# Oneflow-Inc/libai

Hardware: AMD Instinct MI355X
Metric: tokens/sec (whole node), GPT-2 345M 3D-parallel at 1/2/4/8 MI355X (higher is better)
Workload: dtype bf16; 1 GPU; model=gpt2-345m (nl24 h1024 nah16 seq1024), global_batch=48, seq_len=1024, parallelism=dp1

## Files before the change

### libai_amd/csrc/bindings.cpp

```cpp
#include <algorithm>
#include <torch/extension.h>
#include <c10/hip/HIPStream.h>
#include <hip/hip_runtime_api.h>

#include <tuple>
#include <vector>

namespace {

hipStream_t cur_stream() { return c10::hip::getCurrentHIPStream().stream(); }

void check_launch(const char* name) {
  hipError_t err = hipGetLastError();
  TORCH_CHECK(err == hipSuccess, name, " launch failed: ", hipGetErrorString(err));
}

bool is_bf16(const torch::Tensor& t) {
  TORCH_CHECK(t.scalar_type() == torch::kBFloat16 || t.scalar_type() == torch::kFloat32,
              "libai_amd kernels support bf16/f32, got ", t.scalar_type());
  return t.scalar_type() == torch::kBFloat16;
}

void check_bias_width(const char* op, int W, int V) {
  TORCH_CHECK(W % V == 0 && W >= V, op, ": width ", W,
// ... 70 lines not shown
                    int64_t,
                    int64_t, int64_t, int64_t, int64_t, int64_t, int64_t, int64_t,
                    int64_t, int64_t, int64_t, int64_t, int64_t, int64_t, int64_t,
                    int64_t, int64_t, int64_t, int64_t, int64_t, int64_t, int64_t,
                    int64_t, int, int, int, int, int, float, float, uint64_t, int,
                    int, const float*, int, const float*, float*, const int*,
                    const int*, hipStream_t);
void attn_dropout_apply_bf16(void*, int64_t, int64_t, int64_t, float, uint64_t,
                             hipStream_t);
void attn_dropout_apply_f32(void*, int64_t, int64_t, int64_t, float, uint64_t,
                            hipStream_t);
void embedding_fwd_bf16(const int64_t*, const void*, void*, int64_t, int64_t,
                        int64_t, int64_t, hipStream_t);
void embedding_fwd_f32(const int64_t*, const void*, void*, int64_t, int64_t,
                       int64_t, int64_t, hipStream_t);
void embedding_bwd_bf16(const int64_t*, const void*, float*, int64_t, int64_t,
                        int64_t, int64_t, int64_t, hipStream_t);
void embedding_bwd_f32(const int64_t*, const void*, float*, int64_t, int64_t,
                       int64_t, int64_t, int64_t, hipStream_t);
void gemm_dw_bf16(const void*, const void*, float*, void*, int, int64_t, int64_t,
                  int64_t, int64_t, hipStream_t);
void flash_decode_bf16(const void*, const void*, const void*, void*, const int*,
                       int64_t, int64_t, int64_t, int64_t, int64_t, int64_t,
                       int64_t, int64_t, int64_t, int64_t, int, int, int, int,
                       float, int, const float*, int, hipStream_t);
int flash_decode_num_splits(int, int, int);
void flash_decode_split_bf16(const void*, const void*, const void*, void*,
                             float*, float*, float*, const int*, int64_t,
                             int64_t, int64_t, int64_t, int64_t, int64_t,
                             int64_t, int64_t, int64_t, int64_t, int, int, int,
                             int, int, float, int, const float*, int,
                             hipStream_t);
void rope_fwd_bf16(const void*, void*, const float*, const float*, int64_t, int64_t,
                   int64_t, int64_t, int64_t, int64_t, int, int, int, int, int,
                   const int*, int, hipStream_t);
void rope_fwd_f32(const void*, void*, const float*, const float*, int64_t, int64_t,
                  int64_t, int64_t, int64_t, int64_t, int, int, int, int, int,
                  const int*, int, hipStream_t);
void rope_bwd_bf16(const void*, void*, const float*, const float*, int64_t, int64_t,
                   int64_t, int64_t, int64_t, int64_t, int, int, int, int, int,
                   const int*, int, hipStream_t);
void rope_bwd_f32(const void*, void*, const float*, const float*, int64_t, int64_t,
                  int64_t, int64_t, int64_t, int64_t, int, int, int, int, int,
                  const int*, int, hipStream_t);
void rope_kv_insert_bf16(const void*, const void*, const void*, void*, void*,
                         void*, const float*, const float*, const long long*,
                         int, int, int, int, int64_t, int64_t, int64_t, int64_t,
                         int64_t, int64_t, int64_t, int, int, hipStream_t);
void quant_fp8_bf16(const void*, void*, const float*, float*, int64_t,
                    hipStream_t);
void res_ln_fwd_bf16(const void*, const void*, const void*, const void*,
                     const void*, void*, void*, int64_t, int, float, bool,
                     hipStream_t);
void swiglu_fwd_bf16(const void*, void*, int64_t, int, hipStream_t);
void swiglu_fwd_f32(const void*, void*, int64_t, int, hipStream_t);
void swiglu_bwd_bf16(const void*, const void*, void*, int64_t, int, hipStream_t);
void swiglu_bwd_f32(const void*, const void*, void*, int64_t, int, hipStream_t);
int adamw_chunk_elems();
void adamw_step_bf16(const void*, int, float, float, float, float, float, float, float,
                     float, hipStream_t);
void adamw_step_f32(const void*, int, float, float, float, float, float, float, float,
                    float, hipStream_t);
void l2norm_sq_bf16(const void*, int, float*, hipStream_t);
void l2norm_sq_f32(const void*, int, float*, hipStream_t);
}

std::tuple<torch::Tensor, torch::Tensor, torch::Tensor> ln_fwd(
    torch::Tensor x, torch::Tensor gamma, c10::optional<torch::Tensor> beta, bool rms,
    double eps) {
  CHECK_IN(x);
  CHECK_IN(gamma);
  const int H = (int)gamma.numel();
  const int64_t R = x.numel() / H;
  auto y = torch::empty_like(x);
  auto opts = x.options().dtype(torch::kFloat32);
  auto mean = rms ? torch::empty({0}, opts) : torch::empty({R}, opts);
  auto rstd = torch::empty({R}, opts);
  const void* bptr = nullptr;
  if (beta.has_value()) {
    CHECK_IN(beta.value());
    bptr = beta->data_ptr();
  }
  auto fn = is_bf16(x) ? ln_fwd_bf16 : ln_fwd_f32;
  fn(x.data_ptr(), gamma.data_ptr(), bptr, y.data_ptr(),
     rms ? nullptr : mean.data_ptr<float>(), rstd.data_ptr<float>(), R, H, (float)eps,
     rms, cur_stream());
  check_launch("ln_fwd");
  return {y, mean, rstd};
}

std::tuple<torch::Tensor, torch::Tensor, torch::Tensor> ln_bwd(
    torch::Tensor dy, torch::Tensor x, torch::Tensor gamma, torch::Tensor mean,
    torch::Tensor rstd, bool rms, bool need_dbeta) {
  CHECK_IN(dy);
  CHECK_IN(x);
  const int H = (int)gamma.numel();
  const int64_t R = x.numel() / H;
  auto dx = torch::empty_like(x);
  auto dgamma = torch::empty_like(gamma);
  auto dbeta = need_dbeta ? torch::empty_like(gamma) : torch::Tensor();
  const int64_t gxw = std::max<int64_t>(1, (H / 8 + 255) / 256);
  const int P = (int)std::min<int64_t>(std::max<int64_t>(1, 1024 / gxw),
                                       std::max<int64_t>(1, R / 4));
  auto partial = torch::empty({(need_dbeta ? 2L : 1L) * P, (int64_t)H},
                              x.options().dtype(torch::kFloat32));
  float* pgamma = partial.data_ptr<float>();
  float* pbeta = need_dbeta ? pgamma + (int64_t)P * H : nullptr;
  auto fdx = is_bf16(x) ? ln_bwd_dx_bf16 : ln_bwd_dx_f32;
  auto fw = is_bf16(x) ? ln_bwd_wgrad_bf16 : ln_bwd_wgrad_f32;
  const float* meanp = rms ? nullptr : mean.data_ptr<float>();
  fdx(dy.data_ptr(), x.data_ptr(), gamma.data_ptr(), meanp, rstd.data_ptr<float>(),
      dx.data_ptr(), R, H, rms, cur_stream());
  fw(dy.data_ptr(), x.data_ptr(), meanp, rstd.data_ptr<float>(), pgamma, pbeta,
     dgamma.data_ptr(), need_dbeta ? dbeta.data_ptr() : nullptr, R, H, P, rms,
     cur_stream());
  check_launch("ln_bwd");
  dgamma.copy_(partial.narrow(0, 0, P).sum(0));
  if (need_dbeta) dbeta.copy_(partial.narrow(0, P, P).sum(0));
  return {dx, dgamma, dbeta};
}

torch::Tensor bias_gelu_fwd(torch::Tensor x, c10::optional<torch::Tensor> b) {
  CHECK_IN(x);
  auto y = torch::empty_like(x);
  const int W = b.has_value() ? (int)b->numel() : (int)x.size(-1);
  check_bias_width("bias_gelu_fwd", W, is_bf16(x) ? 8 : 4);
  auto fn = is_bf16(x) ? bias_gelu_fwd_bf16 : bias_gelu_fwd_f32;
  fn(x.data_ptr(), b.has_value() ? b->data_ptr() : nullptr, y.data_ptr(), x.numel(), W,
     cur_stream());
  check_launch("bias_gelu_fwd");
  return y;
}

std::tuple<torch::Tensor, c10::optional<torch::Tensor>> bias_gelu_bwd(
    torch::Tensor x, c10::optional<torch::Tensor> b, torch::Tensor dy,
    bool want_dbias) {
  CHECK_IN(x);
  CHECK_IN(dy);
  auto dx = torch::empty_like(x);
  const int W = b.has_value() ? (int)b->numel() : (int)x.size(-1);
  const int V = is_bf16(x) ? 8 : 4;
  check_bias_width("bias_gelu_bwd", W, V);
  float* pp = nullptr;
  torch::Tensor partial;
  int P = 0;
  if (want_dbias) {
    P = bias_col_grid_rows(x.numel(), W, V);
    partial = torch::empty({P, W}, x.options().dtype(torch::kFloat32));
    pp = partial.data_ptr<float>();
  }
  auto fn = is_bf16(x) ? bias_gelu_bwd_bf16 : bias_gelu_bwd_f32;
  fn(x.data_ptr(), b.has_value() ? b->data_ptr() : nullptr, dy.data_ptr(), dx.data_ptr(),
     pp, x.numel(), W, cur_stream());
  check_launch("bias_gelu_bwd");
  if (pp != nullptr)
    return {dx, partial.sum(0).to(x.scalar_type())};
  return {dx, c10::nullopt};
}

torch::Tensor colsum(torch::Tensor x, int64_t W) {
  CHECK_IN(x);
  const int64_t R = x.numel() / W;
  const int64_t gxw = std::max<int64_t>(1, (W / 8 + 255) / 256);
  const int P = (int)std::min<int64_t>(std::max<int64_t>(1, 1024 / gxw),
                                       std::max<int64_t>(1, R / 4));
  auto partial = torch::empty({P, W}, x.options().dtype(torch::kFloat32));
  auto out = torch::empty({W}, x.options());
  auto fn = is_bf16(x) ? colsum_bf16 : colsum_f32;
  fn(x.data_ptr(), partial.data_ptr<float>(), out.data_ptr(), R, (int)W, P,
     cur_stream());
  check_launch("colsum");
  out.copy_(partial.sum(0));
// ... 485 lines not shown
  auto out = torch::empty(x.sizes(),
                          x.options().dtype(torch::kFloat8_e4m3fn));
  quant_fp8_bf16(x.data_ptr(), out.data_ptr(), scale.data_ptr<float>(),
                 amax.data_ptr<float>(), x.numel(), cur_stream());
  check_launch("quant_fp8");
  return out;
}

torch::Tensor swiglu_fwd(torch::Tensor x) {
  CHECK_IN(x);
  const int64_t F = x.size(-1) / 2;
  auto sizes = x.sizes().vec();
  sizes.back() = F;
  auto y = torch::empty(sizes, x.options());
  auto fn = is_bf16(x) ? swiglu_fwd_bf16 : swiglu_fwd_f32;
  fn(x.data_ptr(), y.data_ptr(), x.numel() / (2 * F), (int)F, cur_stream());
  check_launch("swiglu_fwd");
  return y;
}

torch::Tensor swiglu_bwd(torch::Tensor x, torch::Tensor dy) {
  CHECK_IN(x);
  CHECK_IN(dy);
  const int64_t F = x.size(-1) / 2;
  auto dx = torch::empty_like(x);
  auto fn = is_bf16(x) ? swiglu_bwd_bf16 : swiglu_bwd_f32;
  fn(x.data_ptr(), dy.data_ptr(), dx.data_ptr(), x.numel() / (2 * F), (int)F,
     cur_stream());
  check_launch("swiglu_bwd");
  return dx;
}

void adamw_step(torch::Tensor chunks, bool bf16_params, double lr, double beta1,
                double beta2, double eps, double wd, double bc1, double bc2,
                double grad_scale) {
  CHECK_IN(chunks);
  TORCH_CHECK(chunks.scalar_type() == torch::kInt64 && chunks.size(1) == 6);
  auto fn = bf16_params ? adamw_step_bf16 : adamw_step_f32;
  fn(chunks.data_ptr(), (int)chunks.size(0), (float)lr, (float)beta1, (float)beta2,
     (float)eps, (float)wd, (float)bc1, (float)bc2, (float)grad_scale, cur_stream());
  check_launch("adamw_step");
}

void l2norm_sq(torch::Tensor chunks, bool bf16_grads, torch::Tensor out) {
  CHECK_IN(chunks);
  TORCH_CHECK(chunks.scalar_type() == torch::kInt64 && chunks.size(1) == 2);
  auto fn = bf16_grads ? l2norm_sq_bf16 : l2norm_sq_f32;
  fn(chunks.data_ptr(), (int)chunks.size(0), out.data_ptr<float>(), cur_stream());
  check_launch("l2norm_sq");
}

PYBIND11_MODULE(TORCH_EXTENSION_NAME, m) {
  m.def("ln_fwd", &ln_fwd);
  m.def("ln_bwd", &ln_bwd);
  m.def("bias_gelu_fwd", &bias_gelu_fwd);
  m.def("bias_gelu_bwd", &bias_gelu_bwd);
  m.def("colsum", &colsum);
  m.def("bias_dropout_res_fwd", &bias_dropout_res_fwd);
  m.def("bias_dropout_res_bwd", &bias_dropout_res_bwd);
  m.def("softmax_fwd", &softmax_fwd);
  m.def("softmax_bwd", &softmax_bwd);
  m.def("lt_gelu_aux_bias", &lt_gelu_aux_bias);
  m.def("lt_dgelu_bgrad", &lt_dgelu_bgrad);
  m.def("lt_epilogues_available", &lt_epilogues_available);
  m.def("gemm_dw", &gemm_dw);
  m.def("flash_decode", &flash_decode, py::arg("q"), py::arg("k"), py::arg("v"),
        py::arg("scale"), py::arg("kv_len"),
        py::arg("alibi_slopes") = py::none(), py::arg("window") = 0);
  m.def("embedding_fwd", &embedding_fwd);
  m.def("embedding_bwd", &embedding_bwd);
  m.def("flash_fwd", &flash_fwd, py::arg("q"), py::arg("k"), py::arg("v"),
        py::arg("scale"), py::arg("p_drop"), py::arg("seed"), py::arg("causal"),
        py::arg("kv_len"), py::arg("alibi_slopes") = py::none(), py::arg("window") = 0,
        py::arg("rel_bias") = py::none(), py::arg("doc_start") = py::none(),
        py::arg("doc_end") = py::none());
  m.def("flash_bwd", &flash_bwd, py::arg("q"), py::arg("k"), py::arg("v"),
        py::arg("o"), py::arg("dout"), py::arg("lse"), py::arg("scale"),
        py::arg("p_drop"), py::arg("seed"), py::arg("causal"), py::arg("dqkv"),
        py::arg("kv_len"), py::arg("alibi_slopes") = py::none(), py::arg("window") = 0,
        py::arg("rel_bias") = py::none(), py::arg("doc_start") = py::none(),
        py::arg("doc_end") = py::none());
  m.def("attn_dropout_apply", &attn_dropout_apply);
  m.def("ce_fwd", &ce_fwd);
  m.def("ce_bwd", &ce_bwd);
  m.def("rope", &rope, py::arg("x"), py::arg("cos_t"), py::arg("sin_t"),
        py::arg("pos0"), py::arg("bwd"), py::arg("pos_ids") = py::none());
  m.def("rope_kv_insert", &rope_kv_insert);
  m.def("quant_fp8", &quant_fp8);
  m.def("res_norm_fwd", &res_norm_fwd);
  m.def("swiglu_fwd", &swiglu_fwd);
  m.def("swiglu_bwd", &swiglu_bwd);
  m.def("adamw_step", &adamw_step);
  m.def("l2norm_sq", &l2norm_sq);
  m.def("adamw_chunk_elems", &adamw_chunk_elems);
}
```

### libai_amd/layers/attention.py

```python

import math

import torch
from torch import nn

from ..ops.fused_bias import bias_dropout_add
from ..ops.softmax import fused_scale_mask_softmax

_DUMMY_TABS = {}


def _dummy_tab(device):
    key = str(device)
    if key not in _DUMMY_TABS:
        _DUMMY_TABS[key] = torch.zeros(1, dtype=torch.float32, device=device)
    return _DUMMY_TABS[key]


def _rel_table_fits(table, num_heads, s, device):
    return (
        table.dtype == torch.float32
        and table.device == device
        and tuple(table.shape) == (num_heads, 2 * s - 1)
    )
# ... 33 lines not shown
        self.head_size = hidden_size // num_attention_heads
        dutil = du.get_dist_util()
        tp = dutil.tensor_parallel_size
        assert num_attention_heads % tp == 0, (num_attention_heads, tp)
        self.num_heads_local = num_attention_heads // tp
        self.attn_mask_type = attn_mask_type
        self.attention_dropout_prob = attention_dropout_prob
        self.output_dropout_prob = output_dropout_prob
        self.layer_idx = layer_idx
        self.is_cross_attention = is_cross_attention
        self.sequence_parallel = sequence_parallel
        assert not (sequence_parallel and is_cross_attention), \
            "sequence parallelism is wired for self-attention blocks only"

        self.norm_factor = 1.0 / math.sqrt(self.head_size)
        self.coeff = None
        if apply_query_key_layer_scaling:
            self.coeff = float(layer_idx + 1)
            self.norm_factor /= self.coeff

        output_layer_init_method = output_layer_init_method or init_method
        if is_cross_attention:
            self.query = Linear1D(hidden_size, hidden_size, parallel="col",
                                  init_method=init_method, layer_idx=layer_idx)
            self.key_value = Linear1D(hidden_size, 2 * hidden_size, parallel="col",
                                      init_method=init_method, layer_idx=layer_idx)
        else:
            self.query_key_value = Linear1D(hidden_size, 3 * hidden_size, parallel="col",
                                            init_method=init_method,
                                            sequence_parallel=sequence_parallel,
                                            layer_idx=layer_idx)
        self.dense = Linear1D(hidden_size, hidden_size, parallel="row",
                              init_method=output_layer_init_method,
                              skip_bias_add=True,
                              sequence_parallel=sequence_parallel,
                              layer_idx=layer_idx)

    def _split_heads(self, x, n):
        b, s, _ = x.shape
        x = x.view(b, s, self.num_heads_local, n * self.head_size)
        return x.permute(0, 2, 1, 3).chunk(n, dim=-1)

    def forward(
        self,
        hidden_states,
        encoder_states=None,
        attention_mask=None,
        past_key_value=None,
        use_cache=False,
        residual=None,
        position_bias=None,
        static_cache=None,
        position=None,
    ):
        if static_cache is not None:
            from ..ops._ext import ext
            from ..ops.attention import flash_decode_attn

            ck, cv, kv_len32 = static_cache
            qkv = self.query_key_value(hidden_states)
            b, s, _ = hidden_states.shape
            nh, hs = self.num_heads_local, self.head_size
            qkv4 = qkv.view(b, s, nh, 3 * hs)
            q, k, v = (qkv4[..., :hs], qkv4[..., hs:2 * hs], qkv4[..., 2 * hs:])
            dummy = _dummy_tab(hidden_states.device)
            qo = ext().rope_kv_insert(q, k, v, ck, cv, dummy, dummy,
                                      position, False)
            scale_c = self.norm_factor * (self.coeff if self.coeff else 1.0)
            ctx = flash_decode_attn(qo, ck, cv, scale_c, kv_len=kv_len32)
            context = ctx.permute(0, 2, 1, 3).reshape(b, 1, nh * hs)
            return self.dense(context)

        from ..ops.attention import bias_alibi_slopes, bias_rel_table

        slopes = bias_alibi_slopes(position_bias)
        bias_fusable = position_bias is None or slopes is not None
        rel_table = bias_rel_table(position_bias) if slopes is None else None

        if (
            not self.is_cross_attention
            and past_key_value is None
            and not use_cache
            and (bias_fusable or rel_table is not None)
        ):
            from ..ops.attention import (
                flash_attention_available,
                flash_attention_qkv,
                mask_kv_len,
            )

            b, s, _ = hidden_states.shape
            if self.sequence_parallel:
                s = s * du.get_dist_util().tensor_parallel_size
            if flash_attention_available(
                self.head_size, hidden_states.dtype, hidden_states.device, s, s,
                attention_mask,
            ) and (rel_table is None or _rel_table_fits(
                rel_table, self.num_heads_local, s, hidden_states.device
            )):
                qkv = self.query_key_value(hidden_states)
                qkv5 = qkv.view(b, s, self.num_heads_local, 3, self.head_size)
                o = flash_attention_qkv(
                    qkv5,
                    scale=self.norm_factor * (self.coeff if self.coeff else 1.0),
                    p_drop=self.attention_dropout_prob,
                    causal=self.attn_mask_type == AttnMaskType.causal,
                    training=self.training,
                    kv_len=mask_kv_len(attention_mask),
                    alibi_slopes=slopes,
                    rel_bias=rel_table,
                )
                context = o.reshape(b, s, self.num_heads_local * self.head_size)
                out, bias = self.dense(context)
                return bias_dropout_add(
                    out, bias=bias, residual=residual, p=self.output_dropout_prob,
                    training=self.training,
                )

        if self.is_cross_attention:
            q = self._split_heads(self.query(hidden_states), 1)[0]
            if past_key_value is not None:
                k, v = past_key_value
            else:
                k, v = self._split_heads(self.key_value(encoder_states), 2)
        else:
            q, k, v = self._split_heads(self.query_key_value(hidden_states), 3)
            if past_key_value is not None:
                pk, pv = past_key_value
                k = torch.cat([pk, k], dim=2)
                v = torch.cat([pv, v], dim=2)
        present = (k, v) if use_cache else None

        scale_d = self.norm_factor * (self.coeff if self.coeff else 1.0)
        if (
            past_key_value is not None
            and attention_mask is None
            and bias_fusable
            and not self.is_cross_attention
        ):
            from ..ops.attention import (
                decode_attention_available,
                flash_decode_attn,
            )

            if decode_attention_available(q, self.head_size):
                ctx = flash_decode_attn(q.contiguous(), k, v, scale_d,
                                        alibi_slopes=slopes)
                b, nh, _, hs = ctx.shape
                context = ctx.permute(0, 2, 1, 3).reshape(b, 1, nh * hs)
                out, bias = self.dense(context)
                out = bias_dropout_add(
                    out, bias=bias, residual=residual,
                    p=self.output_dropout_prob, training=self.training,
                )
                return (out, present) if use_cache else out

        scores = torch.matmul(q, k.transpose(-1, -2))
        scale = self.norm_factor * (self.coeff if self.coeff else 1.0)
        if position_bias is not None:
            scores = scores * scale + position_bias
            scale = 1.0
        causal = self.attn_mask_type == AttnMaskType.causal and past_key_value is None
        probs = fused_scale_mask_softmax(
            scores,
            pad_mask=attention_mask,
            scale=scale,
            p=self.attention_dropout_prob,
            causal=causal,
            training=self.training,
        )
        context = torch.matmul(probs, v)
        b, nh, sq, hs = context.shape
        context = context.permute(0, 2, 1, 3).reshape(b, sq, nh * hs)

        out, bias = self.dense(context)
        out = bias_dropout_add(
            out, bias=bias, residual=residual, p=self.output_dropout_prob,
            training=self.training,
        )
        if use_cache:
            return out, present
        return out

    def extra_repr(self):
        return (
            f"hidden_size={self.hidden_size}, num_heads={self.num_heads}, "
            f"layer_idx={self.layer_idx}, mask={self.attn_mask_type}"
        )
```

### libai_amd/layers/transformer_layer.py

```python

import torch
from torch import nn

from .attention import AttnMaskType, MultiheadAttention
from .layer_norm import LayerNorm
from .mlp import MLP

__all__ = ["TransformerLayer"]


class TransformerLayer(nn.Module):
    def __init__(
        self,
        hidden_size,
        ffn_hidden_size,
        num_attention_heads,
        is_decoder=False,
        attention_dropout_prob=0.0,
        output_dropout_prob=0.0,
        layernorm_epsilon=1e-5,
        init_method=nn.init.xavier_normal_,
        output_layer_init_method=None,
        bias_gelu_fusion=True,
        bias_dropout_fusion=True,
        scale_mask_softmax_fusion=True,
        apply_query_key_layer_scaling=False,
        apply_residual_post_layernorm=False,
        attn_mask_type=AttnMaskType.padding,
        mlp_type="dense",
        activation="gelu",
        sequence_parallel=False,
        moe_num_experts=8,
        moe_top_k=2,
        *,
        layer_idx=0,
    ):
        super().__init__()
        self.layer_idx = layer_idx
        self.is_decoder = is_decoder
        self.apply_residual_post_layernorm = apply_residual_post_layernorm
        self.sequence_parallel = sequence_parallel
        assert not (sequence_parallel and is_decoder), \
            "sequence parallelism: encoder/causal self-attention blocks only"
        assert not (sequence_parallel and mlp_type == "gated"), \
            "sequence parallelism + gated MLP not wired yet"
        output_layer_init_method = output_layer_init_method or init_method
        self._sp = sequence_parallel

        self.input_layernorm = LayerNorm(hidden_size, eps=layernorm_epsilon,
                                         layer_idx=layer_idx)
        self.self_attention = MultiheadAttention(
            hidden_size, num_attention_heads,
            attention_dropout_prob=attention_dropout_prob,
            output_dropout_prob=output_dropout_prob,
            init_method=init_method,
            output_layer_init_method=output_layer_init_method,
            bias_dropout_fusion=bias_dropout_fusion,
            scale_mask_softmax_fusion=scale_mask_softmax_fusion,
            apply_query_key_layer_scaling=apply_query_key_layer_scaling,
            attn_mask_type=attn_mask_type,
            sequence_parallel=sequence_parallel,
            layer_idx=layer_idx,
        )
        self.post_attention_layernorm = LayerNorm(hidden_size, eps=layernorm_epsilon,
                                                  layer_idx=layer_idx)
        if is_decoder:
            self.cross_attention = MultiheadAttention(
                hidden_size, num_attention_heads, is_cross_attention=True,
                attention_dropout_prob=attention_dropout_prob,
                output_dropout_prob=output_dropout_prob,
                init_method=init_method,
                output_layer_init_method=output_layer_init_method,
                attn_mask_type=AttnMaskType.padding,
                layer_idx=layer_idx,
            )
            self.post_cross_attention_layernorm = LayerNorm(
                hidden_size, eps=layernorm_epsilon, layer_idx=layer_idx
            )
        if mlp_type == "moe":
            from .moe import MoELayer

            assert not sequence_parallel, "MoE + SP not wired yet"
            self.mlp = MoELayer(
                hidden_size, ffn_hidden_size, num_experts=moe_num_experts,
                top_k=moe_top_k, activation=activation,
                init_method=init_method,
                output_layer_init_method=output_layer_init_method,
                layer_idx=layer_idx,
            )
        elif mlp_type == "gated":
            from .mlp import GatedMLP

            self.mlp = GatedMLP(
                hidden_size, ffn_hidden_size,
                output_dropout_prob=output_dropout_prob,
                activation=activation,
                init_method=init_method,
                output_layer_init_method=output_layer_init_method,
                layer_idx=layer_idx,
            )
        else:
            self.mlp = MLP(
                hidden_size, ffn_hidden_size,
                output_dropout_prob=output_dropout_prob,
                init_method=init_method,
                output_layer_init_method=output_layer_init_method,
                bias_gelu_fusion=bias_gelu_fusion,
                bias_dropout_fusion=bias_dropout_fusion,
                activation=activation,
                sequence_parallel=sequence_parallel,
                layer_idx=layer_idx,
            )
        if sequence_parallel:
            for ln in (self.input_layernorm, self.post_attention_layernorm):
                for p in ln.parameters():
                    p.sequence_parallel_grad = True

    def forward(
        self,
        hidden_states,
        attention_mask=None,
        encoder_states=None,
        encoder_attention_mask=None,
        past_key_value=None,
        use_cache=False,
        position_bias=None,
        static_cache=None,
        position=None,
    ):
        if static_cache is not None:
            from ..ops._ext import ext
            from ..ops.fused_bias import bias_dropout_add

            ln1 = self.input_layernorm(hidden_states)
            residual = ln1 if self.apply_residual_post_layernorm else hidden_states
            out, bias = self.self_attention(ln1, residual=residual,
                                            static_cache=static_cache,
                                            position=position)
            ln = self.post_attention_layernorm
            if out.shape[-1] <= 2048:
                h, ln2 = ext().res_norm_fwd(out, bias, residual, ln.weight,
                                            ln.bias, ln.eps, False)
            else:
                h = bias_dropout_add(out, bias=bias, residual=residual,
                                     p=0.0, training=False)
                ln2 = ln(h)
            residual = ln2 if self.apply_residual_post_layernorm else h
            return self.mlp(ln2, residual=residual)
        if past_key_value is not None:
            if self.is_decoder:
                self_past, cross_past = past_key_value
            else:
                self_past, cross_past = past_key_value, None
        else:
            self_past, cross_past = None, None

        ln1 = self.input_layernorm(hidden_states)
        residual = ln1 if self.apply_residual_post_layernorm else hidden_states
        attn_out = self.self_attention(
            ln1, attention_mask=attention_mask, past_key_value=self_past,
            use_cache=use_cache, residual=residual, position_bias=position_bias,
        )
        if use_cache:
            attn_out, self_present = attn_out
        hidden_states = attn_out

        presents = None
        if self.is_decoder and encoder_states is not None:
            ln_c = self.post_attention_layernorm(hidden_states)
            residual = ln_c if self.apply_residual_post_layernorm else hidden_states
            cross_out = self.cross_attention(
                ln_c, encoder_states=encoder_states,
                attention_mask=encoder_attention_mask, past_key_value=cross_past,
                use_cache=use_cache, residual=residual,
            )
            if use_cache:
                cross_out, cross_present = cross_out
                presents = (self_present, cross_present)
            hidden_states = cross_out
            ln2 = self.post_cross_attention_layernorm(hidden_states)
        else:
            if use_cache:
                presents = self_present
            ln2 = self.post_attention_layernorm(hidden_states)

        residual = ln2 if self.apply_residual_post_layernorm else hidden_states
        out = self.mlp(ln2, residual=residual)
        if use_cache:
            return out, presents
        return out
```

### libai_amd/ops/__init__.py

```python
from ._ext import draw_seed, ext, has_ext, use_hip
from .attention import flash_attention, flash_attention_available
from .cross_entropy import vocab_parallel_cross_entropy
from .fused_bias import bias_dropout_add, bias_gelu
from .norm import layer_norm, rms_norm
from .rope import RotaryEmbedding, apply_rotary_pos_emb
from .softmax import fused_scale_mask_softmax
from .swiglu import swiglu

__all__ = [
    "ext",
    "has_ext",
    "use_hip",
    "draw_seed",
    "layer_norm",
    "rms_norm",
    "bias_gelu",
    "bias_dropout_add",
    "fused_scale_mask_softmax",
    "vocab_parallel_cross_entropy",
    "flash_attention",
    "flash_attention_available",
    "apply_rotary_pos_emb",
    "RotaryEmbedding",
    "swiglu",
]
```

### libai_amd/ops/norm.py

```python

import torch
import torch.nn.functional as F

from ._ext import ext, use_hip

__all__ = ["layer_norm", "rms_norm"]


class _NormFn(torch.autograd.Function):
    @staticmethod
    def forward(ctx, x, weight, bias, eps, rms):
        x = x.contiguous()
        y, mean, rstd = ext().ln_fwd(x, weight.contiguous(),
                                     bias.contiguous() if bias is not None else None,
                                     rms, eps)
        ctx.save_for_backward(x, weight, mean, rstd)
        ctx.rms = rms
        ctx.has_bias = bias is not None
        return y

    @staticmethod
    def backward(ctx, dy):
        x, weight, mean, rstd = ctx.saved_tensors
        dx, dgamma, dbeta = ext().ln_bwd(
            dy.contiguous(), x, weight, mean, rstd, ctx.rms, ctx.has_bias
        )
        return dx, dgamma, (dbeta if ctx.has_bias else None), None, None


def layer_norm(x, weight, bias, eps=1e-5):
    if use_hip(x):
        return _NormFn.apply(x, weight, bias, eps, False)
    return F.layer_norm(x, (weight.numel(),), weight, bias, eps)


def _rms_norm_ref(x, weight, eps):
    dt = x.dtype
    xf = x.float()
    rstd = torch.rsqrt(xf.pow(2).mean(-1, keepdim=True) + eps)
    return (xf * rstd).to(dt) * weight


def rms_norm(x, weight, eps=1e-5):
    if use_hip(x):
        return _NormFn.apply(x, weight, None, eps, True)
    return _rms_norm_ref(x, weight, eps)
```

Measured before the change: 299,000 tokens/s.

## Fuse bias-dropout-residual-add with LayerNorm and single-pass norm backward

Adds HIP kernels that fuse the attention output bias, dropout, residual add and the following LayerNorm into one wave-per-row kernel, with a matching fused backward. The backward computes dx, dgamma/dbeta/dbias partials and the residual gradient in one pass. The standard ln_bwd also gains a single-pass fused path that accumulates the residual gradient in-kernel instead of a separate add. The transformer layer routes through these fused ops by default for non-decoder, non-SP training. This is meant to cut kernel launches and extra activation reads and writes. In exchange it adds a per-block partial reduction that is folded with a torch sum, and dropout masks are regenerated from a hash.

```diff
diff --git a/libai_amd/csrc/bindings.cpp b/libai_amd/csrc/bindings.cpp
--- a/libai_amd/csrc/bindings.cpp
+++ b/libai_amd/csrc/bindings.cpp
@@ -146,6 +146,20 @@
 void res_ln_fwd_bf16(const void*, const void*, const void*, const void*,
                      const void*, void*, void*, int64_t, int, float, bool,
                      hipStream_t);
+bool norm_wave_path(int, int);
+int norm_bwd_fused_blocks(int64_t);
+int ln_bwd_fused_bf16(const void*, const void*, const void*, const float*,
+                       const float*, const void*, void*, float*, bool, int64_t, int,
+                       int, bool, hipStream_t);
+int ln_bwd_fused_f32(const void*, const void*, const void*, const float*,
+                      const float*, const void*, void*, float*, bool, int64_t, int,
+                      int, bool, hipStream_t);
+void res_drop_ln_fwd_bf16(const void*, const void*, const void*, const void*,
+                          const void*, void*, void*, float*, float*, int64_t, int,
+                          float, bool, float, uint64_t, hipStream_t);
+int res_drop_ln_bwd_bf16(const void*, const void*, const void*, const float*,
+                          const float*, const void*, void*, void*, float*, bool, bool,
+                          int64_t, int, int, bool, float, uint64_t, hipStream_t);
 void swiglu_fwd_bf16(const void*, void*, int64_t, int, hipStream_t);
 void swiglu_fwd_f32(const void*, void*, int64_t, int, hipStream_t);
 void swiglu_bwd_bf16(const void*, const void*, void*, int64_t, int, hipStream_t);
@@ -185,12 +199,35 @@
 
 std::tuple<torch::Tensor, torch::Tensor, torch::Tensor> ln_bwd(
     torch::Tensor dy, torch::Tensor x, torch::Tensor gamma, torch::Tensor mean,
-    torch::Tensor rstd, bool rms, bool need_dbeta) {
+    torch::Tensor rstd, bool rms, bool need_dbeta, c10::optional<torch::Tensor> dres,
+    bool single_pass) {
   CHECK_IN(dy);
   CHECK_IN(x);
   const int H = (int)gamma.numel();
   const int64_t R = x.numel() / H;
   auto dx = torch::empty_like(x);
+  if (dres.has_value()) {
+    CHECK_IN(dres.value());
+    TORCH_CHECK(dres->numel() == x.numel() && dres->scalar_type() == x.scalar_type(),
+                "ln_bwd: dres must match x");
+  }
+  if (single_pass && R > 0 && norm_wave_path(H, is_bf16(x) ? 8 : 4)) {
+    const int maxP = norm_bwd_fused_blocks(R);
+    const int64_t K = need_dbeta ? 2 : 1;
+    auto partial =
+        torch::empty({(int64_t)maxP, K * H}, x.options().dtype(torch::kFloat32));
+    auto fn = is_bf16(x) ? ln_bwd_fused_bf16 : ln_bwd_fused_f32;
+    const int P = fn(dy.data_ptr(), x.data_ptr(), gamma.data_ptr(),
+       rms ? nullptr : mean.data_ptr<float>(), rstd.data_ptr<float>(),
+       dres.has_value() ? dres->data_ptr() : nullptr, dx.data_ptr(),
+       partial.data_ptr<float>(), need_dbeta, R, H, maxP, rms, cur_stream());
+    check_launch("ln_bwd_fused");
+    auto folded = partial.narrow(0, 0, P).sum(0);
+    auto dg = folded.narrow(0, 0, H).to(gamma.scalar_type());
+    auto dbt = need_dbeta ? folded.narrow(0, H, H).to(gamma.scalar_type())
+                          : torch::Tensor();
+    return {dx, dg, dbt};
+  }
   auto dgamma = torch::empty_like(gamma);
   auto dbeta = need_dbeta ? torch::empty_like(gamma) : torch::Tensor();
   const int64_t gxw = std::max<int64_t>(1, (H / 8 + 255) / 256);
@@ -211,7 +248,92 @@
   check_launch("ln_bwd");
   dgamma.copy_(partial.narrow(0, 0, P).sum(0));
   if (need_dbeta) dbeta.copy_(partial.narrow(0, P, P).sum(0));
+  if (dres.has_value()) dx.add_(dres->view_as(dx));
   return {dx, dgamma, dbeta};
+}
+
+std::vector<torch::Tensor> res_drop_norm_fwd(
+    torch::Tensor x, c10::optional<torch::Tensor> bias, torch::Tensor res,
+    torch::Tensor gamma, c10::optional<torch::Tensor> beta, double eps, bool rms,
+    double p, int64_t seed) {
+  CHECK_IN(x);
+  CHECK_IN(res);
+  CHECK_IN(gamma);
+  TORCH_CHECK(x.scalar_type() == torch::kBFloat16, "res_drop_norm_fwd: bf16 only");
+  const int H = (int)x.size(-1);
+  TORCH_CHECK(norm_wave_path(H, 8), "res_drop_norm_fwd: width ", H,
+              " is outside the wave path");
+  TORCH_CHECK(res.numel() == x.numel() && res.scalar_type() == x.scalar_type() &&
+                  gamma.numel() == H && gamma.scalar_type() == x.scalar_type(),
+              "res_drop_norm_fwd: res / gamma must match x");
+  const void* bp = nullptr;
+  const void* btp = nullptr;
+  if (bias.has_value()) {
+    CHECK_IN(bias.value());
+    TORCH_CHECK(bias->numel() == H && bias->scalar_type() == x.scalar_type());
+    bp = bias->data_ptr();
+  }
+  if (beta.has_value()) {
+    CHECK_IN(beta.value());
+    TORCH_CHECK(beta->numel() == H && beta->scalar_type() == x.scalar_type());
+    btp = beta->data_ptr();
+  }
+  const int64_t R = x.numel() / H;
+  auto h = torch::empty_like(x);
+  auto y = torch::empty_like(x);
+  auto opts = x.options().dtype(torch::kFloat32);
+  auto mean = rms ? torch::empty({0}, opts) : torch::empty({R}, opts);
+  auto rstd = torch::empty({R}, opts);
+  if (R > 0) {
+    res_drop_ln_fwd_bf16(x.data_ptr(), bp, res.data_ptr(), gamma.data_ptr(), btp,
+                         h.data_ptr(), y.data_ptr(),
+                         rms ? nullptr : mean.data_ptr<float>(), rstd.data_ptr<float>(),
+                         R, H, (float)eps, rms, (float)p, (uint64_t)seed, cur_stream());
+    check_launch("res_drop_norm_fwd");
+  }
+  return {h, y, mean, rstd};
+}
+
+std::vector<torch::Tensor> res_drop_norm_bwd(
+    torch::Tensor dy, torch::Tensor h, torch::Tensor gamma, torch::Tensor mean,
+    torch::Tensor rstd, c10::optional<torch::Tensor> dres, bool rms, bool need_dbeta,
+    bool want_dbias, double p, int64_t seed) {
+  CHECK_IN(dy);
+  CHECK_IN(h);
+  CHECK_IN(gamma);
+  TORCH_CHECK(h.scalar_type() == torch::kBFloat16, "res_drop_norm_bwd: bf16 only");
+  const int H = (int)h.size(-1);
+  TORCH_CHECK(norm_wave_path(H, 8) && gamma.numel() == H,
+              "res_drop_norm_bwd: width ", H, " is outside the wave path");
+  TORCH_CHECK(dy.numel() == h.numel() && dy.scalar_type() == h.scalar_type(),
+              "res_drop_norm_bwd: dy must match h");
+  if (dres.has_value()) {
+    CHECK_IN(dres.value());
+    TORCH_CHECK(dres->numel() == h.numel() && dres->scalar_type() == h.scalar_type(),
+                "res_drop_norm_bwd: dres must match h");
+  }
+  const int64_t R = h.numel() / H;
+  TORCH_CHECK(R > 0, "res_drop_norm_bwd: empty input");
+  TORCH_CHECK(rstd.numel() == R && (rms || mean.numel() == R));
+  auto dh = torch::empty_like(h);
+  auto dx = p > 0 ? torch::empty_like(h) : dh;
+  const int maxP = norm_bwd_fused_blocks(R);
+  const int64_t K = 1 + (need_dbeta ? 1 : 0) + (want_dbias ? 1 : 0);
+  auto partial =
+      torch::empty({(int64_t)maxP, K * H}, h.options().dtype(torch::kFloat32));
+  const int P = res_drop_ln_bwd_bf16(dy.data_ptr(), h.data_ptr(), gamma.data_ptr(),
+                       rms ? nullptr : mean.data_ptr<float>(), rstd.data_ptr<float>(),
+                       dres.has_value() ? dres->data_ptr() : nullptr, dh.data_ptr(),
+                       dx.data_ptr(), partial.data_ptr<float>(), need_dbeta, want_dbias,
+                       R, H, maxP, rms, (float)p, (uint64_t)seed, cur_stream());
+  check_launch("res_drop_norm_bwd");
+  auto folded = partial.narrow(0, 0, P).sum(0);
+  auto dg = folded.narrow(0, 0, H).to(h.scalar_type());
+  auto dbt = need_dbeta ? folded.narrow(0, H, H).to(h.scalar_type()) : torch::Tensor();
+  auto dbs = want_dbias ? folded.narrow(0, (need_dbeta ? 2 : 1) * (int64_t)H, H)
+                              .to(h.scalar_type())
+                        : torch::Tensor();
+  return {dh, dx, dg, dbt, dbs};
 }
 
 torch::Tensor bias_gelu_fwd(torch::Tensor x, c10::optional<torch::Tensor> b) {
@@ -803,7 +925,11 @@
 
 PYBIND11_MODULE(TORCH_EXTENSION_NAME, m) {
   m.def("ln_fwd", &ln_fwd);
-  m.def("ln_bwd", &ln_bwd);
+  m.def("ln_bwd", &ln_bwd, py::arg("dy"), py::arg("x"), py::arg("gamma"),
+        py::arg("mean"), py::arg("rstd"), py::arg("rms"), py::arg("need_dbeta"),
+        py::arg("dres") = py::none(), py::arg("single_pass") = true);
+  m.def("res_drop_norm_fwd", &res_drop_norm_fwd);
+  m.def("res_drop_norm_bwd", &res_drop_norm_bwd);
   m.def("bias_gelu_fwd", &bias_gelu_fwd);
   m.def("bias_gelu_bwd", &bias_gelu_bwd);
   m.def("colsum", &colsum);
diff --git a/libai_amd/csrc/kernels/res_norm.hip b/libai_amd/csrc/kernels/res_norm.hip
--- /dev/null
+++ b/libai_amd/csrc/kernels/res_norm.hip
@@ -0,0 +1,403 @@
+#include "common.h"
+
+#pragma clang fp contract(off)
+
+namespace {
+
+template <int V>
+__device__ __forceinline__ void drop_keep(float (&keep)[V], uint64_t seed,
+                                          uint64_t vec_idx, uint32_t thr8,
+                                          float scale) {
+#pragma unroll
+  for (int q = 0; q < V / 4; ++q) {
+    const uint32_t h = rnd_hash(seed, vec_idx * (V / 4) + q);
+#pragma unroll
+    for (int j = 0; j < 4; ++j)
+      keep[q * 4 + j] = (((h >> (j * 8)) & 0xFFu) >= thr8) ? scale : 0.f;
+  }
+}
+
+template <class E, bool RMS, int NV, bool DROP, bool BIAS>
+__global__ void res_drop_norm_fwd_wave_kernel(
+    const typename E::T* __restrict__ x, const typename E::T* __restrict__ bias,
+    const typename E::T* __restrict__ res, const typename E::T* __restrict__ gamma,
+    const typename E::T* __restrict__ beta, typename E::T* __restrict__ h,
+    typename E::T* __restrict__ y, float* __restrict__ mean_out,
+    float* __restrict__ rstd_out, int H, float eps, int64_t R, float p,
+    uint64_t seed) {
+  using T = typename E::T;
+  using VecT = typename E::VecT;
+  constexpr int V = E::VEC;
+  const int wave = threadIdx.x >> 6;
+  const int lane = threadIdx.x & 63;
+  const int64_t row = (int64_t)blockIdx.x * (blockDim.x >> 6) + wave;
+  if (row >= R) return;
+  const T* xr = x + row * (int64_t)H;
+  const T* rr = res + row * (int64_t)H;
+  T* hr = h + row * (int64_t)H;
+  T* yr = y + row * (int64_t)H;
+  const int nvec = H / V;
+  const float scale = 1.0f / (1.0f - p);
+  const uint32_t thr8 = drop_threshold_u8(p);
+
+  VecT vh[NV];
+  float sum = 0.f, sumsq = 0.f;
+#pragma unroll
+  for (int n = 0; n < NV; ++n) {
+    const int i = lane + n * 64;
+    if (i < nvec) {
+      VecT vx = ((const VecT*)xr)[i];
+      VecT vr = ((const VecT*)rr)[i];
+      VecT vb;
+      if (BIAS) vb = ((const VecT*)bias)[i];
+      float keep[V];
+      if (DROP) drop_keep<V>(keep, seed, (uint64_t)(row * nvec + i), thr8, scale);
+#pragma unroll
+      for (int j = 0; j < V; ++j) {
+        const float v = E::to_f(vx[j]) + (BIAS ? E::to_f(vb[j]) : 0.f);
+        vh[n][j] = E::from_f(DROP ? __builtin_fmaf(v, keep[j], E::to_f(vr[j]))
+                                  : v + E::to_f(vr[j]));
+        const float g = E::to_f(vh[n][j]);
+        sum += g;
+        sumsq += g * g;
+      }
+      ((VecT*)hr)[i] = vh[n];
+    }
+  }
+#pragma unroll
+  for (int off = 32; off > 0; off >>= 1) {
+    sum += __shfl_xor(sum, off, 64);
+    sumsq += __shfl_xor(sumsq, off, 64);
+  }
+  const float mean = RMS ? 0.f : sum / H;
+  const float rstd =
+      rsqrtf((RMS ? sumsq / H : __builtin_fmaf(-mean, mean, sumsq / H)) + eps);
+  if (lane == 0) {
+    if (!RMS) mean_out[row] = mean;
+    rstd_out[row] = rstd;
+  }
+#pragma unroll
+  for (int n = 0; n < NV; ++n) {
+    const int i = lane + n * 64;
+    if (i < nvec) {
+      VecT g = ((const VecT*)gamma)[i];
+      VecT o;
+      if (!RMS && beta != nullptr) {
+        VecT b = ((const VecT*)beta)[i];
+#pragma unroll
+        for (int j = 0; j < V; ++j)
+          o[j] = E::from_f(__builtin_fmaf((E::to_f(vh[n][j]) - mean) * rstd,
+                                          E::to_f(g[j]), E::to_f(b[j])));
+      } else {
+#pragma unroll
+        for (int j = 0; j < V; ++j)
+          o[j] = E::from_f((E::to_f(vh[n][j]) - mean) * rstd * E::to_f(g[j]));
+      }
+      ((VecT*)yr)[i] = o;
+    }
+  }
+}
+
+template <class E, bool RMS, int NV, bool DRES, bool DROP, bool DBIAS>
+__global__ void __launch_bounds__(256) norm_bwd_fused_wave_kernel(
+    const typename E::T* __restrict__ dy, const typename E::T* __restrict__ x,
+    const typename E::T* __restrict__ gamma, const float* __restrict__ mean_in,
+    const float* __restrict__ rstd_in, const typename E::T* __restrict__ dres,
+    typename E::T* __restrict__ dh, typename E::T* __restrict__ dxd,
+    float* __restrict__ partial, bool wbeta, int H, int64_t R, float p,
+    uint64_t seed) {
+  using T = typename E::T;
+  using VecT = typename E::VecT;
+  constexpr int V = E::VEC;
+  constexpr int HV = V / 4;
+  extern __shared__ __attribute__((aligned(16))) float red[];
+  f32x4* red4 = (f32x4*)red;
+
+  const int wave = threadIdx.x >> 6;
+  const int lane = threadIdx.x & 63;
+  const int nw = blockDim.x >> 6;
+  const int nvec = H / V;
+  const float scale = 1.0f / (1.0f - p);
+  const uint32_t thr8 = drop_threshold_u8(p);
+
+  VecT vg[NV];
+  float dg[NV][V], db[NV][V], dbi[DBIAS ? NV : 1][V];
+#pragma unroll
+  for (int n = 0; n < NV; ++n) {
+    const int i = lane + n * 64;
+    if (i < nvec) vg[n] = ((const VecT*)gamma)[i];
+#pragma unroll
+    for (int j = 0; j < V; ++j) {
+      dg[n][j] = 0.f;
+      db[n][j] = 0.f;
+      if (DBIAS) dbi[n][j] = 0.f;
+    }
+  }
+
+  for (int64_t row = (int64_t)blockIdx.x * nw + wave; row < R;
+       row += (int64_t)gridDim.x * nw) {
+    const T* dyr = dy + row * (int64_t)H;
+    const T* xr = x + row * (int64_t)H;
+    const float mean = RMS ? 0.f : mean_in[row];
+    const float rstd = rstd_in[row];
+
+    VecT vdy[NV], vx[NV], vdr[DRES ? NV : 1];
+    float s1 = 0.f, s2 = 0.f;
+#pragma unroll
+    for (int n = 0; n < NV; ++n) {
+      const int i = lane + n * 64;
+      if (i < nvec) {
+        vdy[n] = ((const VecT*)dyr)[i];
+        vx[n] = ((const VecT*)xr)[i];
+        if (DRES) vdr[n] = ((const VecT*)(dres + row * (int64_t)H))[i];
+#pragma unroll
+        for (int j = 0; j < V; ++j) {
+          const float dyg = E::to_f(vdy[n][j]) * E::to_f(vg[n][j]);
+          const float xhat = (E::to_f(vx[n][j]) - mean) * rstd;
+          s1 += dyg;
+          s2 += dyg * xhat;
+        }
+      }
+    }
+#pragma unroll
+    for (int off = 32; off > 0; off >>= 1) {
+      s1 += __shfl_xor(s1, off, 64);
+      s2 += __shfl_xor(s2, off, 64);
+    }
+    s1 /= H;
+    s2 /= H;
+#pragma unroll
+    for (int n = 0; n < NV; ++n) {
+      const int i = lane + n * 64;
+      if (i < nvec) {
+        float keep[V];
+        if (DROP) drop_keep<V>(keep, seed, (uint64_t)(row * nvec + i), thr8, scale);
+        VecT o, od;
+#pragma unroll
+        for (int j = 0; j < V; ++j) {
+          const float dyv = E::to_f(vdy[n][j]);
+          const float xhat = (E::to_f(vx[n][j]) - mean) * rstd;
+          constexpr bool kRmsFmaOnS2 = sizeof(T) == 4 && NV == 2;
+          const float gj = E::to_f(vg[n][j]);
+          const float u =
+              !RMS ? __builtin_fmaf(-xhat, s2, __builtin_fmaf(dyv, gj, -s1))
+              : kRmsFmaOnS2 ? __builtin_fmaf(-xhat, s2, dyv * gj)
+                            : __builtin_fmaf(dyv, gj, -(xhat * s2));
+          o[j] = E::from_f(rstd * u);
+          if (DRES) o[j] = E::from_f(E::to_f(o[j]) + E::to_f(vdr[n][j]));
+          dg[n][j] += dyv * (E::to_f(vx[n][j]) - mean) * rstd;
+          db[n][j] += dyv;
+          if (DROP) {
+            const float g = E::to_f(o[j]) * keep[j];
+            od[j] = E::from_f(g);
+            if (DBIAS) dbi[n][j] += g;
+          } else if (DBIAS) {
+            dbi[n][j] += E::to_f(o[j]);
+          }
+        }
+        ((VecT*)(dh + row * (int64_t)H))[i] = o;
+        if (DROP) ((VecT*)(dxd + row * (int64_t)H))[i] = od;
+      }
+    }
+  }
+
+  const int kbeta = 1, kbias = wbeta ? 2 : 1;
+  for (int w = 0; w < nw; ++w) {
+    if (wave == w) {
+#pragma unroll
+      for (int n = 0; n < NV; ++n) {
+#pragma unroll
+        for (int q = 0; q < HV; ++q) {
+          const int s0 = (n * HV + q) * 64 + lane;
+          const int sb = ((kbeta * NV + n) * HV + q) * 64 + lane;
+          const int sx = ((kbias * NV + n) * HV + q) * 64 + lane;
+          f32x4 a = {dg[n][q * 4], dg[n][q * 4 + 1], dg[n][q * 4 + 2],
+                     dg[n][q * 4 + 3]};
+          if (w > 0) a = red4[s0] + a;
+          red4[s0] = a;
+          if (wbeta) {
+            f32x4 b = {db[n][q * 4], db[n][q * 4 + 1], db[n][q * 4 + 2],
+                       db[n][q * 4 + 3]};
+            if (w > 0) b = red4[sb] + b;
+            red4[sb] = b;
+          }
+          if (DBIAS) {
+            f32x4 c = {dbi[n][q * 4], dbi[n][q * 4 + 1], dbi[n][q * 4 + 2],
+                       dbi[n][q * 4 + 3]};
+            if (w > 0) c = red4[sx] + c;
+            red4[sx] = c;
+          }
+        }
+      }
+    }
+    __syncthreads();
+  }
+  const int K = 1 + (wbeta ? 1 : 0) + (DBIAS ? 1 : 0);
+  const int H4 = H / 4;
+  f32x4* prow = (f32x4*)(partial + (int64_t)blockIdx.x * K * H);
+  for (int c = threadIdx.x; c < K * H4; c += blockDim.x) {
+    const int k = c / H4, c4 = c - k * H4;
+    const int i = c4 / HV, q = c4 - i * HV;
+    prow[c] = red4[((k * NV + (i >> 6)) * HV + q) * 64 + (i & 63)];
+  }
+}
+
+constexpr int kBwdThreads = 256;
+constexpr int kBwdMaxBlocks = 1024;
+
+template <class E, bool RMS, int NV, bool DRES, bool DROP, bool DBIAS>
+int launch_bwd_inst(const void* dy, const void* x, const void* gamma,
+                    const float* mean, const float* rstd, const void* dres,
+                    void* dh, void* dxd, float* partial, bool wbeta, int64_t R,
+                    int H, int maxP, float p, uint64_t seed, hipStream_t stream) {
+  using T = typename E::T;
+  auto kern = norm_bwd_fused_wave_kernel<E, RMS, NV, DRES, DROP, DBIAS>;
+  const size_t lds = (size_t)3 * NV * E::VEC * 64 * sizeof(float);
+  static int resident = 0;
+  if (resident == 0) {
+    int dev = 0, cus = 0, per = 0;
+    if (hipGetDevice(&dev) != hipSuccess ||
+        hipDeviceGetAttribute(&cus, hipDeviceAttributeMultiprocessorCount, dev) !=
+            hipSuccess ||
+        hipOccupancyMaxActiveBlocksPerMultiprocessor(&per, kern, kBwdThreads, lds) !=
+            hipSuccess)
+      cus = per = 0;
+    resident = cus * per > 0 ? cus * per : kBwdMaxBlocks;
+  }
+  const int P = resident < maxP ? resident : maxP;
+  kern<<<dim3(P), dim3(kBwdThreads), lds, stream>>>(
+      (const T*)dy, (const T*)x, (const T*)gamma, mean, rstd, (const T*)dres, (T*)dh,
+      (T*)dxd, partial, wbeta, H, R, p, seed);
+  return P;
+}
+
+template <class E, bool RMS, int NV, bool DROP, bool DBIAS>
+int launch_bwd_dres(const void* dy, const void* x, const void* gamma,
+                     const float* mean, const float* rstd, const void* dres,
+                     void* dh, void* dxd, float* partial, bool wbeta, int64_t R,
+                     int H, int P, float p, uint64_t seed, hipStream_t stream) {
+  if (dres != nullptr)
+    return launch_bwd_inst<E, RMS, NV, true, DROP, DBIAS>(
+        dy, x, gamma, mean, rstd, dres, dh, dxd, partial, wbeta, R, H, P, p, seed,
+        stream);
+  return launch_bwd_inst<E, RMS, NV, false, DROP, DBIAS>(
+      dy, x, gamma, mean, rstd, dres, dh, dxd, partial, wbeta, R, H, P, p, seed,
+      stream);
+}
+
+template <class E, bool DROP, bool DBIAS>
+int launch_bwd(const void* dy, const void* x, const void* gamma, const float* mean,
+                const float* rstd, const void* dres, void* dh, void* dxd,
+                float* partial, bool wbeta, int64_t R, int H, int P, bool rms,
+                float p, uint64_t seed, hipStream_t stream) {
+  const int nvl = CDIV(H / E::VEC, 64);
+#define BWD_NV(RMS_, NV_)                                                     \
+  return launch_bwd_dres<E, RMS_, NV_, DROP, DBIAS>(dy, x, gamma, mean, rstd, \
+                                                    dres, dh, dxd, partial,   \
+                                                    wbeta, R, H, P, p, seed,  \
+                                                    stream)
+#define BWD_RMS(RMS_)  \
+  if (nvl <= 1)        \
+    BWD_NV(RMS_, 1);   \
+  else if (nvl == 2)   \
+    BWD_NV(RMS_, 2);   \
+  else                 \
+    BWD_NV(RMS_, 4)
+  if (rms) {
+    BWD_RMS(true);
+  } else {
+    BWD_RMS(false);
+  }
+#undef BWD_RMS
+#undef BWD_NV
+}
+
+template <class E, bool RMS, bool DROP, bool BIAS>
+void launch_fwd(const void* x, const void* bias, const void* res, const void* gamma,
+                const void* beta, void* h, void* y, float* mean, float* rstd,
+                int64_t R, int H, float eps, float p, uint64_t seed,
+                hipStream_t stream) {
+  using T = typename E::T;
+  const int nvl = CDIV(H / E::VEC, 64);
+  dim3 g((uint32_t)CDIV(R, 4));
+#define FWD_NV(NV_)                                                              \
+  res_drop_norm_fwd_wave_kernel<E, RMS, NV_, DROP, BIAS>                         \
+      <<<g, dim3(256), 0, stream>>>((const T*)x, (const T*)bias, (const T*)res,  \
+                                    (const T*)gamma, (const T*)beta, (T*)h,      \
+                                    (T*)y, mean, rstd, H, eps, R, p, seed)
+  if (nvl <= 1)
+    FWD_NV(1);
+  else if (nvl == 2)
+    FWD_NV(2);
+  else
+    FWD_NV(4);
+#undef FWD_NV
+}
+
+}
+
+extern "C" bool norm_wave_path(int H, int vec) {
+  return H >= vec && H % vec == 0 && CDIV(H / vec, 64) <= 4;
+}
+
+extern "C" int norm_bwd_fused_blocks(int64_t R) {
+  const int64_t g = CDIV(R, (int64_t)(kBwdThreads / 64));
+  return (int)(g < kBwdMaxBlocks ? (g < 1 ? 1 : g) : kBwdMaxBlocks);
+}
+
+#define NORM_BWD_FUSED(SUFF, ETYPE)                                              \
+  extern "C" int ln_bwd_fused_##SUFF(                                            \
+      const void* dy, const void* x, const void* gamma, const float* mean,       \
+      const float* rstd, const void* dres, void* dx, float* partial, bool wbeta, \
+      int64_t R, int H, int P, bool rms, hipStream_t stream) {                   \
+    return launch_bwd<ETYPE, false, false>(dy, x, gamma, mean, rstd, dres, dx,   \
+                                           nullptr, partial, wbeta, R, H, P,     \
+                                           rms, 0.f, 0, stream);                 \
+  }
+
+NORM_BWD_FUSED(bf16, BF16Elem)
+NORM_BWD_FUSED(f32, F32Elem)
+
+extern "C" void res_drop_ln_fwd_bf16(const void* x, const void* bias, const void* res,
+                                     const void* gamma, const void* beta, void* h,
+                                     void* y, float* mean, float* rstd, int64_t R,
+                                     int H, float eps, bool rms, float p,
+                                     uint64_t seed, hipStream_t stream) {
+#define FWD_ARGS x, bias, res, gamma, beta, h, y, mean, rstd, R, H, eps, p, seed, stream
+#define FWD_SEL(RMS_)                                      \
+  if (p > 0.f) {                                           \
+    if (bias)                                              \
+      launch_fwd<BF16Elem, RMS_, true, true>(FWD_ARGS);    \
+    else                                                   \
+      launch_fwd<BF16Elem, RMS_, true, false>(FWD_ARGS);   \
+  } else {                                                 \
+    if (bias)                                              \
+      launch_fwd<BF16Elem, RMS_, false, true>(FWD_ARGS);   \
+    else                                                   \
+      launch_fwd<BF16Elem, RMS_, false, false>(FWD_ARGS);  \
+  }
+  if (rms) {
+    FWD_SEL(true)
+  } else {
+    FWD_SEL(false)
+  }
+#undef FWD_SEL
+#undef FWD_ARGS
+}
+
+extern "C" int res_drop_ln_bwd_bf16(const void* dy, const void* h, const void* gamma,
+                                     const float* mean, const float* rstd,
+                                     const void* dres, void* dh, void* dxd,
+                                     float* partial, bool wbeta, bool wbias,
+                                     int64_t R, int H, int P, bool rms, float p,
+                                     uint64_t seed, hipStream_t stream) {
+#define BWD_ARGS \
+  dy, h, gamma, mean, rstd, dres, dh, dxd, partial, wbeta, R, H, P, rms, p, seed, stream
+  if (p > 0.f) {
+    if (wbias) return launch_bwd<BF16Elem, true, true>(BWD_ARGS);
+    return launch_bwd<BF16Elem, true, false>(BWD_ARGS);
+  }
+  if (wbias) return launch_bwd<BF16Elem, false, true>(BWD_ARGS);
+  return launch_bwd<BF16Elem, false, false>(BWD_ARGS);
+#undef BWD_ARGS
+}
diff --git a/libai_amd/layers/attention.py b/libai_amd/layers/attention.py
--- a/libai_amd/layers/attention.py
+++ b/libai_amd/layers/attention.py
@@ -109,7 +109,9 @@
         position_bias=None,
         static_cache=None,
         position=None,
+        raw_output=False,
     ):
+        assert not raw_output or (past_key_value is None and not use_cache)
         if static_cache is not None:
             from ..ops._ext import ext
             from ..ops.attention import flash_decode_attn
@@ -169,6 +171,8 @@
                 )
                 context = o.reshape(b, s, self.num_heads_local * self.head_size)
                 out, bias = self.dense(context)
+                if raw_output:
+                    return out, bias
                 return bias_dropout_add(
                     out, bias=bias, residual=residual, p=self.output_dropout_prob,
                     training=self.training,
@@ -231,6 +235,8 @@
         context = context.permute(0, 2, 1, 3).reshape(b, sq, nh * hs)
 
         out, bias = self.dense(context)
+        if raw_output:
+            return out, bias
         out = bias_dropout_add(
             out, bias=bias, residual=residual, p=self.output_dropout_prob,
             training=self.training,
diff --git a/libai_amd/layers/transformer_layer.py b/libai_amd/layers/transformer_layer.py
--- a/libai_amd/layers/transformer_layer.py
+++ b/libai_amd/layers/transformer_layer.py
@@ -34,9 +34,11 @@
         moe_top_k=2,
         *,
         layer_idx=0,
+        fuse_residual_norm=True,
     ):
         super().__init__()
         self.layer_idx = layer_idx
+        self.fuse_residual_norm = fuse_residual_norm
         self.is_decoder = is_decoder
         self.apply_residual_post_layernorm = apply_residual_post_layernorm
         self.sequence_parallel = sequence_parallel
@@ -116,6 +118,18 @@
                 for p in ln.parameters():
                     p.sequence_parallel_grad = True
 
+    def _fuse_residual_chain(self, past_key_value, use_cache):
+        return (
+            self.fuse_residual_norm
+            and not self.apply_residual_post_layernorm
+            and not self.is_decoder
+            and not self._sp
+            and not use_cache
+            and past_key_value is None
+            and self.input_layernorm.weight is not None
+            and self.post_attention_layernorm.weight is not None
+        )
+
     def forward(
         self,
         hidden_states,
@@ -155,6 +169,22 @@
         else:
             self_past, cross_past = None, None
 
+        if self._fuse_residual_chain(past_key_value, use_cache):
+            from ..ops.norm import bias_dropout_add_norm, layer_norm_residual
+
+            ln_in, ln = self.input_layernorm, self.post_attention_layernorm
+            ln1, residual = layer_norm_residual(hidden_states, ln_in.weight,
+                                                ln_in.bias, ln_in.eps)
+            out, bias = self.self_attention(
+                ln1, attention_mask=attention_mask, position_bias=position_bias,
+                raw_output=True,
+            )
+            h, ln2 = bias_dropout_add_norm(
+                out, bias, residual, ln.weight, ln.bias, ln.eps,
+                p=self.self_attention.output_dropout_prob, training=self.training,
+            )
+            return self.mlp(ln2, residual=h)
+
         ln1 = self.input_layernorm(hidden_states)
         residual = ln1 if self.apply_residual_post_layernorm else hidden_states
         attn_out = self.self_attention(
diff --git a/libai_amd/ops/__init__.py b/libai_amd/ops/__init__.py
--- a/libai_amd/ops/__init__.py
+++ b/libai_amd/ops/__init__.py
@@ -2,7 +2,12 @@
 from .attention import flash_attention, flash_attention_available
 from .cross_entropy import vocab_parallel_cross_entropy
 from .fused_bias import bias_dropout_add, bias_gelu
-from .norm import layer_norm, rms_norm
+from .norm import (
+    bias_dropout_add_norm,
+    layer_norm,
+    layer_norm_residual,
+    rms_norm,
+)
 from .rope import RotaryEmbedding, apply_rotary_pos_emb
 from .softmax import fused_scale_mask_softmax
 from .swiglu import swiglu
@@ -14,6 +19,8 @@
     "draw_seed",
     "layer_norm",
     "rms_norm",
+    "layer_norm_residual",
+    "bias_dropout_add_norm",
     "bias_gelu",
     "bias_dropout_add",
     "fused_scale_mask_softmax",
diff --git a/libai_amd/ops/norm.py b/libai_amd/ops/norm.py
--- a/libai_amd/ops/norm.py
+++ b/libai_amd/ops/norm.py
@@ -2,9 +2,11 @@
 import torch
 import torch.nn.functional as F
 
-from ._ext import ext, use_hip
+from ._ext import draw_seed, ext, use_hip
+from .fused_bias import bias_dropout_add
 
-__all__ = ["layer_norm", "rms_norm"]
+__all__ = ["layer_norm", "rms_norm", "layer_norm_residual",
+           "bias_dropout_add_norm", "res_norm_fusable"]
 
 
 class _NormFn(torch.autograd.Function):
@@ -45,3 +47,96 @@
     if use_hip(x):
         return _NormFn.apply(x, weight, None, eps, True)
     return _rms_norm_ref(x, weight, eps)
+
+
+class _NormResFn(torch.autograd.Function):
+
+    @staticmethod
+    def forward(ctx, x, weight, bias, eps, rms):
+        assert x.is_contiguous()
+        y, mean, rstd = ext().ln_fwd(x, weight.contiguous(),
+                                     bias.contiguous() if bias is not None else None,
+                                     rms, eps)
+        ctx.save_for_backward(x, weight, mean, rstd)
+        ctx.rms = rms
+        ctx.has_bias = bias is not None
+        ctx.set_materialize_grads(False)
+        return y, x
+
+    @staticmethod
+    def backward(ctx, dy, dres):
+        if dy is None:
+            return dres, None, None, None, None
+        x, weight, mean, rstd = ctx.saved_tensors
+        dx, dgamma, dbeta = ext().ln_bwd(
+            dy.contiguous(), x, weight, mean, rstd, ctx.rms, ctx.has_bias,
+            dres.contiguous() if dres is not None else None,
+        )
+        return dx, dgamma, (dbeta if ctx.has_bias else None), None, None
+
+
+def layer_norm_residual(x, weight, bias, eps=1e-5, rms=False):
+    if use_hip(x) and x.is_contiguous():
+        return _NormResFn.apply(x, weight, bias, eps, rms)
+    y = rms_norm(x, weight, eps) if rms else layer_norm(x, weight, bias, eps)
+    return y, x
+
+
+def res_norm_fusable(x, weight):
+    H = x.shape[-1]
+    return (
+        use_hip(x)
+        and x.dtype == torch.bfloat16
+        and weight is not None
+        and weight.dtype == torch.bfloat16
+        and H % 8 == 0
+        and 8 <= H <= 2048
+        and x.numel() > 0
+    )
+
+
+class _BiasDropoutAddNormFn(torch.autograd.Function):
+    @staticmethod
+    def forward(ctx, x, bias, residual, weight, beta, eps, rms, p):
+        x = x.contiguous()
+        b = bias.contiguous() if bias is not None else None
+        bt = beta.contiguous() if beta is not None else None
+        seed = draw_seed() if p > 0 else 0
+        h, y, mean, rstd = ext().res_drop_norm_fwd(
+            x, b, residual.contiguous(), weight.contiguous(), bt, eps, rms, p, seed
+        )
+        ctx.save_for_backward(h, weight, mean, rstd)
+        ctx.p = p
+        ctx.seed = seed
+        ctx.rms = rms
+        ctx.has_bias = b is not None
+        ctx.has_beta = bt is not None
+        ctx.set_materialize_grads(False)
+        return h, y
+
+    @staticmethod
+    def backward(ctx, dres, dy):
+        h, weight, mean, rstd = ctx.saved_tensors
+        if dy is None:
+            if dres is None:
+                return (None,) * 8
+            dy = torch.zeros_like(h)
+        dh, dx, dgamma, dbeta, dbias = ext().res_drop_norm_bwd(
+            dy.contiguous(), h, weight.contiguous(), mean, rstd,
+            dres.contiguous() if dres is not None else None,
+            ctx.rms, ctx.has_beta, ctx.has_bias, ctx.p, ctx.seed,
+        )
+        return dx, dbias, dh, dgamma, dbeta, None, None, None
+
+
+def bias_dropout_add_norm(x, bias, residual, weight, norm_bias, eps=1e-5, p=0.0,
+                          training=True, rms=False):
+    if res_norm_fusable(x, weight):
+        return _BiasDropoutAddNormFn.apply(
+            x, bias, residual, weight, None if rms else norm_bias, eps, rms,
+            p if training else 0.0,
+        )
+    h = bias_dropout_add(x, bias=bias, residual=residual, p=p, training=training)
+    if rms:
+        return h, rms_norm(h, weight, eps)
+    return h, layer_norm(h, weight, norm_bias, eps)
```

New measurement: 306,500 tokens/s (median of 6 runs). +2.5%, better.
